# SelennLamson/AntsRL

Hardware: AMD Instinct MI355X
Metric: ant-steps/sec (ants x envs x steps/s), 256^2 grid (higher is better)
Workload: dtype f64 ant kinematics / f32 grids

## Files before the change

antsrl_amd/build.py:

```python
from __future__ import annotations

import os
import shutil
import subprocess
import sys

HERE = os.path.dirname(os.path.abspath(__file__))
CSRC = os.path.join(HERE, "csrc")
LIB_DIR = os.path.join(HERE, "lib")
LIB_PATH = os.path.join(LIB_DIR, "libantsrl_hip.so")
SOURCES = ["antsrl_act.hip", "antsrl_perceive.hip", "antsrl_update.hip", "antsrl_sweep.hip", "antsrl_state.hip",
           "antsrl_capi.hip", "antsrl_policy.hip", "antsrl_mem.hip",
           "antsrl_memnet.hip", "antsrl_memnet_f32.hip", "antsrl_memtrain.hip", "antsrl_memagent.hip",
           "antsrl_memapi.hip", "antsrl_lintrain.hip", "antsrl_exptrain.hip", "antsrl_linapi.hip",
           "antsrl_rework.hip", "antsrl_reworktrain.hip", "antsrl_reworkapi.hip", "antsrl_monitor.hip", "antsrl_recorder.hip",
           "antsrl_render.hip", "antsrl_stats.hip"]
HEADERS = [os.path.join(CSRC, h) for h in ("antsrl_device.h", "antsrl_util.h", "antsrl_update_env.h",
                                           "antsrl_update_one.h", "antsrl_flush.h", "antsrl_layout.h",
                                           "antsrl_lds_optin.h", "antsrl_fail.h", "antsrl_memnet.h",
                                           "antsrl_memnet_dev.h", "antsrl_memtrain.h", "antsrl_memagent.h", "antsrl_draw.h",
                                           "antsrl_adam.h", "antsrl_dqn.h", "antsrl_dqn_dev.h", "antsrl_lintrain.h",
                                           "antsrl_exptrain.h", "antsrl_rework.h", "antsrl_reworktrain.h", "antsrl_monitor.h",
                                           "antsrl_cellread.h", "antsrl_recorder.h", "antsrl_render.h", "antsrl_stats.h")] + [
    os.path.join(HERE, "..", "include", "antsrl.h")]
FLAGS = ["--offload-arch=gfx950", "-O3", "-ffp-contract=off", "-fPIC", "-shared", "-std=c++17",
         "-Wall", "-Wno-unused-function"]


def hipcc() -> str:
    for cand in (shutil.which("hipcc"), "/opt/rocm/bin/hipcc"):
        if cand and os.path.exists(cand):
            return cand
    raise RuntimeError("hipcc not found (needs the ROCm toolchain)")


HOST_ONLY_SOURCES = ("antsrl_capi.hip", "antsrl_mem.hip", "antsrl_memapi.hip", "antsrl_linapi.hip",
                     "antsrl_reworkapi.hip")


def source_hash() -> str:
    import hashlib
    h = hashlib.sha256()
    for path in sorted([os.path.join(CSRC, s) for s in SOURCES if s not in HOST_ONLY_SOURCES] + [os.path.normpath(x) for x in HEADERS]):
        h.update(os.path.basename(path).encode())
        h.update(open(path, "rb").read())
    return h.hexdigest()[:16]


def is_stale(path: str = LIB_PATH) -> bool:
    if not os.path.exists(path):
        return True
    t = os.path.getmtime(path)
    deps = [os.path.join(CSRC, s) for s in SOURCES] + HEADERS + [os.path.abspath(__file__)]
    return any(os.path.getmtime(d) > t for d in deps)


def build_hip(force: bool = False, verbose: bool = False) -> str:
    if not force and not is_stale():
        return LIB_PATH
    objdir = os.path.join(LIB_DIR, "obj_libantsrl_hip")
    os.makedirs(objdir, exist_ok=True)
    flags = [f for f in FLAGS if f != "-shared"]
    procs = []
    for src in SOURCES:
        obj = os.path.join(objdir, src.replace(".hip", ".o"))
        cmd = [hipcc()] + flags + ["-c", os.path.join(CSRC, src), "-o", obj]
        if verbose:
            print(" ".join(cmd))
        procs.append((subprocess.Popen(cmd), obj, cmd))
    objs = []
    for pr, obj, cmd in procs:
        if pr.wait() != 0:
            raise subprocess.CalledProcessError(pr.returncode, cmd)
        objs.append(obj)
    subprocess.check_call([hipcc(), "--offload-arch=gfx950", "-shared", "-fPIC"] + objs + ["-o", LIB_PATH])
    return LIB_PATH


if __name__ == "__main__":
    print(build_hip(force="--force" in sys.argv, verbose=True))
```

antsrl_amd/csrc/antsrl_update_one.h:

```cpp
#pragma once
#include "antsrl_util.h"
#include "antsrl_update_env.h"

__host__ __device__ inline size_t update_one_lds_bytes(int HT, int R, int nwaves, int N)
{
    return align_up(8 * (size_t)HT, 16) + 48 * (size_t)(R > 0 ? R : 1) + 8 * (size_t)nwaves +
           align_up(4 * (size_t)nwaves, 8) + 16 * (size_t)N + align_up(4 * (size_t)R, 16) + 16;
}

template <int C, bool FWD_REC = false>
__device__ __forceinline__ void update_one_body(const KP &p, const int e, const double *__restrict__ wall_jitter, const int out_buf,
                                                unsigned char *smem, const double g_dep, const double inv_g_dep, UmFwd *fw = nullptr)
{
    const int tid = threadIdx.x, T = blockDim.x;
    const int lane = tid & 63, wave = __builtin_amdgcn_readfirstlane(tid >> 6), nwaves = T >> 6;
    const int N = p.N, W = p.W, H = p.H, R = p.R;
    const size_t G = (size_t)W * H, eN = (size_t)e * N;
    uint32_t *hkeys = (uint32_t *)smem, *hvals = hkeys + p.HT;
    double *rock = (double *)(smem + align_up(8 * (size_t)p.HT, 16));
    double *rk = rock + 4 * (R > 0 ? R : 1);
    double *red = rk + 2 * (R > 0 ? R : 1);
    uint32_t *wave_tot = (uint32_t *)(red + nwaves);
    double *sx = (double *)((unsigned char *)wave_tot + align_up(4 * (size_t)nwaves, 8)), *sy = sx + N;
    uint32_t *rk_hit = (uint32_t *)(sy + N);

    const uint32_t *walls = p.s.walls_bits + (size_t)e * p.words;
    const FoodView food{p.s.food + (size_t)e * G * p.fs, p.fs};
    const size_t PS = (size_t)p.ps;
    float *out = p.s.phero[out_buf] + (size_t)e * G * PS;
    const bool on = tid < N;
    const size_t a = eN + (on ? tid : 0);

    double x = p.s.x[a], y = p.s.y[a];
    const double px0 = STP_LD(p.s.prev_x[a]), py0 = STP_LD(p.s.prev_y[a]);
    const uint8_t rstate = STP_LD(p.s.reward_state[a]);
    const double theta0 = p.s.theta[a];
    float act[C];
#pragma unroll
    for (int c = 0; c < C; ++c) act[c] = STP_LD(p.s.activation[a * C + c]);
    const int32_t wc_l = STP_LD(p.s.walldep_cell[a]), dc_l = STP_LD(p.s.dirty_cell[a]);
    const int32_t wc = (p.scaled && on) ? wc_l : -1;
    const int32_t dc = on ? dc_l : -1;
    const int ts = p.s.timestep[e] + 1;
    if (tid < R) {
        rock[4 * tid + 0] = p.s.rock_cx[(size_t)e * R + tid];
        rock[4 * tid + 1] = p.s.rock_cy[(size_t)e * R + tid];
        rock[4 * tid + 2] = p.s.rock_r[(size_t)e * R + tid];
        rock[4 * tid + 3] = p.s.rock_w[(size_t)e * R + tid];
    }
    for (int h = tid; h < p.HT; h += T) {
        hkeys[h] = HASH_EMPTY;
        hvals[h] = 0u;
    }
    const float food_dc_l = food[dc_l >= 0 ? dc_l : 0];
    const float food_dc = dc >= 0 ? food_dc_l : 0.0f;

    const bool hit = on && test_bit(walls, (uint32_t)((int)x * H + (int)y));
    double u = 0.0;
    if (wall_jitter) {
        uint32_t tot;
        const uint32_t rank = block_excl_scan_flag(hit, wave_tot, lane, wave, nwaves, &tot);
        if (hit) u = wall_jitter[eN + rank];
    } else if (hit) {
        u = jitter_u01(p.rng_seed, p.env_id_base + (uint32_t)e, (uint32_t)ts, (uint32_t)tid);
    }
    bool moved = hit;
    if (hit) {
        x = px0;
        y = py0;
        if (!fw) p.s.theta[a] = theta0 + (u - 0.5);
    }
    if (fw) fw->th = hit ? theta0 + (u - 0.5) : theta0;

    if (R > 0) {
        if (on) {
            sx[tid] = x;
            sy[tid] = y;
        }
        __syncthreads();
        for (int q = wave; q < R; q += nwaves) {
            const double cx = rock[4 * q + 0], cy = rock[4 * q + 1], rad = rock[4 * q + 2];
            const double rad2_hi = rad * rad * (1.0 + 1e-12) + 1e-300;
            double sumx = 0.0, sumy = 0.0;
            bool any = false;
            for (int base = 0; base < N; base += 64) {
                const int i = base + lane;
                double px = 0.0, py = 0.0;
                bool col = false;
                if (i < N) {
                    const double vx = cx - sx[i], vy = cy - sy[i];
                    const double d2 = vx * vx + vy * vy;
                    if (!(d2 > rad2_hi)) {
                        const double d = sqrt(d2);
                        const double f = 1 - rad / (d + 0.001);
                        px = vx * f; py = vy * f;
                        col = !(d > rad);
                    }
                }
                unsigned long long m = __ballot(col);
                any |= m != 0;
                while (m) {
                    const int l = __builtin_ctzll(m);
                    m &= m - 1;
                    sumx += __shfl(px, l);
                    sumy += __shfl(py, l);
                }
            }
            if (lane == 0) {
                rk[2 * q + 0] = cx - sumx / rock[4 * q + 3];
                rk[2 * q + 1] = cy - sumy / rock[4 * q + 3];
                rk_hit[q] = any ? 1u : 0u;
            }
        }
        __syncthreads();
        if (tid < R) {
            p.s.rock_cx[(size_t)e * R + tid] = rk[2 * tid + 0];
            p.s.rock_cy[(size_t)e * R + tid] = rk[2 * tid + 1];
        }
        double ax = 0.0, ay = 0.0;
        for (int q = 0; q < R; ++q) {
            if (!rk_hit[q]) continue;
            const double vx = rk[2 * q + 0] - x, vy = rk[2 * q + 1] - y;
            const double rad = rock[4 * q + 2];
            const double d2 = vx * vx + vy * vy;
            if (d2 > rad * rad * (1.0 + 1e-12) + 1e-300) continue;
            const double d = sqrt(d2);
            const double f = 1 - rad / (d + 0.001);
            double px = vx * f, py = vy * f;
            if (d > rad) { px = 0.0; py = 0.0; }
            ax += px; ay += py;
        }
        x = warp_coord(x + ax, (double)W);
        y = warp_coord(y + ay, (double)H);
        moved = true;
    }

    __syncthreads();
    const uint32_t cell_id = (uint32_t)((int)x * H + (int)y);
    const uint32_t cell = prec_xy(p, (int)x, (int)y);
    float pold[C];
    constexpr bool fw_rec = FWD_REC && C == 2;
    if constexpr (fw_rec) {
        const stream_f4 rec = *reinterpret_cast<const stream_f4 *>(out + (size_t)cell * 4);
        pold[0] = rec.x;
        pold[C - 1] = rec.y;
        fw->food = rec.z;
        fw->meta = __float_as_uint(rec.w);
    } else {
#pragma unroll
        for (int c = 0; c < C; ++c) pold[c] = out[(size_t)cell * PS + c];
    }
    if (fw) {
        double th = fw->th;
        if (fw->has_rot) th = np_mod_d(th + (double)fw->rot * p.max_rot_speed, 2 * PI_D);
        fw->th_new = th;
        sincos(th, &fw->sn, &fw->cs);
        fw->pre = 1;
        fw->ts = ts;
        if (fw->frm_off) {
            double st2, ct2;
            sincos(th + PI_D * 0.5, &st2, &ct2);
            double *fs = reinterpret_cast<double *>(smem + fw->frm_off) + 2 * tid;
            fs[0] = ct2;
            fs[1] = st2;
        }
    }
    if (on) {
        if (moved && !fw) {
            p.s.x[a] = x;
            p.s.y[a] = y;
        }
        STP_ST(p.s.prev_x[a], x);
        STP_ST(p.s.prev_y[a], y);
        if (fw) {
            fw->x = x;
            fw->y = y;
        }
        lww_insert(hkeys, hvals, (uint32_t)p.HT - 1, cell, (uint32_t)tid);
        STP_ST(p.s.reward_state[a], (uint8_t)((double)rstate * 0.9));
    }
    __syncthreads();
    if (p.scaled) {
        if (wc >= 0) {
            for (int c = 0; c < C; ++c) out[(size_t)wc * PS + c] = 0.0f;
            p.s.walldep_cell[a] = -1;
        }
        __syncthreads();
    }
    if constexpr (fw_rec) {
        asm volatile("" : "+v"(pold[0]), "+v"(pold[C - 1]), "+v"(fw->food), "+v"(fw->meta));
    }
    double gain = 0.0;
    if (on) {
        const bool winner = lww_winner(hkeys, hvals, (uint32_t)p.HT - 1, cell) == (uint32_t)tid;
        if (fw && winner) fw->m |= UMFWD_WIN;
        if (winner) {
            if (!p.scaled) {
#pragma unroll
                for (int c = 0; c < C; ++c) {
                    if (act[c] != 0.0f) {
                        float v = pold[c] + act[c];
                        if (p.has_max_val) v = fminf(v, (float)p.max_val);
                        out[(size_t)cell * PS + c] = v;
                    }
                }
            } else {
                bool on_wall;
                if constexpr (fw_rec) on_wall = (fw->meta & META_WALL) != 0;
                else on_wall = test_bit(walls, cell_id);
                bool wrote = false;
#pragma unroll
                for (int c = 0; c < C; ++c) {
                    if (act[c] != 0.0f) {
                        double v = (double)pold[c] * g_dep;
                        if (v < p.threshold || on_wall) v = 0.0;
                        v += (double)act[c];
                        if (p.has_max_val) v = fmin(v, p.max_val);
                        out[(size_t)cell * PS + c] = (float)(v * inv_g_dep);
                        wrote = true;
                    } else if (on_wall) {
                        out[(size_t)cell * PS + c] = 0.0f;
                    }
                }
                if (on_wall && wrote) p.s.walldep_cell[a] = (int32_t)cell;
            }
        }
        if (dc >= 0) {
            gain = (double)food_dc;
            food[dc] = 0.0f;
            p.s.dirty_cell[a] = -1;
        }
    }
    for (int o = 32; o > 0; o >>= 1) gain += __shfl_down(gain, o);
    if (lane == 0) red[wave] = gain;
    __syncthreads();
    if (tid == 0) {
        double s2 = 0.0;
        for (int w = 0; w < nwaves; ++w) s2 += red[w];
        if (s2 != 0.0) p.s.anthill_food[e] += s2;
        p.s.timestep[e] = ts;
    }
}
```

antsrl_amd/csrc/antsrl_util.h:

```cpp
#pragma once
#include <hip/hip_runtime.h>
#include <stdint.h>
#include <stdlib.h>
#include "antsrl_device.h"
#include "antsrl_layout.h"
#include "antsrl_lds_optin.h"

#define WAVE 64
#define PI_D 3.141592653589793
#define HASH_EMPTY 0xFFFFFFFFu

struct FoodView {
    float *b;
    int st;
    __device__ __forceinline__ float &operator[](size_t g) const { return b[g * (size_t)st]; }
};

__device__ __forceinline__ uint32_t prec_xy(const KP &p, const int x, const int y)
{
    return p.tiled ? tiled_slot(x, y, p.H) : (uint32_t)(x * p.H + y);
}
__device__ __forceinline__ uint32_t frec_xy(const KP &p, const int x, const int y)
{
    return p.tiled ? tiled_slot(x, y, p.H) : p.ftile ? tiled44_slot(x, y, p.H) : (uint32_t)(x * p.H + y);
}
__device__ __forceinline__ uint32_t prec_cell(const KP &p, const uint32_t cell)
{
    if (!p.tiled) return cell;
    const uint32_t x = cell / (uint32_t)p.H;
    return prec_xy(p, (int)x, (int)(cell - x * (uint32_t)p.H));
}
__device__ __forceinline__ uint32_t frec_cell(const KP &p, const uint32_t cell)
{
    if (!p.tiled && !p.ftile) return cell;
    const uint32_t x = cell / (uint32_t)p.H;
    return frec_xy(p, (int)x, (int)(cell - x * (uint32_t)p.H));
}

__device__ __forceinline__ double np_mod_d(double a, double b)
{
    double r = fmod(a, b);
    if (r != 0.0) {
        if ((b < 0) != (r < 0)) r += b;
    } else {
        r = copysign(0.0, b);
    }
    return r;
}

__device__ __forceinline__ double warp_coord(double v, double size)
{
    double r = np_mod_d(v, size);
    if (r >= size) r = 0.0;
    return r;
}

__device__ __forceinline__ int wrap_index(int v, int n)
{
    if (v < 0 || v >= n) {
        v %= n;
        if (v < 0) v += n;
    }
    return v;
}

__device__ __forceinline__ bool test_bit(const uint32_t *bits, uint32_t cell)
{
    return (bits[cell >> 5] >> (cell & 31)) & 1u;
}

__device__ __forceinline__ uint64_t mix64(uint64_t z)
{
    z ^= z >> 30; z *= 0xBF58476D1CE4E5B9ULL;
    z ^= z >> 27; z *= 0x94D049BB133111EBULL;
    z ^= z >> 31;
    return z;
}

__device__ __forceinline__ double jitter_u01(uint64_t seed, uint32_t env, uint32_t timestep, uint32_t ant)
{
    uint64_t k = mix64(seed + 0x9E3779B97F4A7C15ULL * ((uint64_t)env + 1));
    k = mix64(k ^ (0xD1B54A32D192ED03ULL * ((uint64_t)timestep + 1)));
    k = mix64(k + 0x9E3779B97F4A7C15ULL * ((uint64_t)ant + 1));
    return (double)(k >> 11) * (1.0 / 9007199254740992.0);
}

__device__ __forceinline__ uint32_t lww_hash(uint32_t cell, uint32_t mask)
{
    return (cell * 2654435761u >> 7) & mask;
}

__device__ __forceinline__ void lww_insert(uint32_t *keys, uint32_t *vals, uint32_t mask, uint32_t cell,
                                           uint32_t ant)
{
    uint32_t h = lww_hash(cell, mask);
    for (;;) {
        uint32_t k = atomicCAS(&keys[h], HASH_EMPTY, cell);
        if (k == HASH_EMPTY || k == cell) {
            atomicMax(&vals[h], ant);
            return;
        }
        h = (h + 1) & mask;
    }
}

__device__ __forceinline__ uint32_t lww_winner(const uint32_t *keys, const uint32_t *vals, uint32_t mask,
                                               uint32_t cell)
{
    uint32_t h = lww_hash(cell, mask);
    while (keys[h] != cell) h = (h + 1) & mask;
    return vals[h];
}

__device__ __forceinline__ void wave_lds_sync()
{
    __builtin_amdgcn_fence(__ATOMIC_ACQ_REL, "wavefront");
    __builtin_amdgcn_wave_barrier();
}

typedef float stream_f4 __attribute__((ext_vector_type(4)));
typedef uint32_t stream_u4 __attribute__((ext_vector_type(4)));
#define ANTSRL_NT_STORE(v, p) __builtin_nontemporal_store(v, p)
__device__ __forceinline__ void store_stream(float *dst, float v) { ANTSRL_NT_STORE(v, dst); }
__device__ __forceinline__ void store_stream(uint16_t *dst, uint16_t v) { ANTSRL_NT_STORE(v, dst); }
__device__ __forceinline__ void store_stream(uint4 *dst, const uint4 &v)
{
    ANTSRL_NT_STORE((stream_u4{v.x, v.y, v.z, v.w}), reinterpret_cast<stream_u4 *>(dst));
}
__device__ __forceinline__ uint16_t bf16_bits(float v) { return __builtin_bit_cast(uint16_t, (__bf16)v); }
__device__ __forceinline__ void store_stream(float4 *dst, const float4 &v)
{
    ANTSRL_NT_STORE((stream_f4{v.x, v.y, v.z, v.w}), reinterpret_cast<stream_f4 *>(dst));
}

#define STP_LD(lv) __builtin_nontemporal_load(&(lv))
#define STP_ST(lv, v) __builtin_nontemporal_store((v), &(lv))

__device__ __forceinline__ double sqrt_lt_threshold(double r)
{
    if (!(r > 0.0)) return 0.0;
    double t = r * r;
    for (int it = 0; it < 8 && sqrt(t) >= r; ++it) t = __longlong_as_double(__double_as_longlong(t) - 1);
    for (int it = 0; it < 16 && sqrt(t) < r; ++it) t = __longlong_as_double(__double_as_longlong(t) + 1);
    return t;
}

__host__ __device__ __forceinline__ size_t align_up(size_t v, size_t a) { return (v + a - 1) / a * a; }

__host__ __device__ inline size_t update_scratch_bytes(int HT, int R, int nwaves)
{
    return align_up(8 * (size_t)HT, 16) + 16 * (size_t)(R > 0 ? R : 1) + 8 * (size_t)nwaves +
           4 * (size_t)nwaves + 16;
}

static inline unsigned grid_for(size_t n)
{
    size_t b = (n + 255) / 256;
    if (b > 65536) b = 65536;
    if (b < 1) b = 1;
    return (unsigned)b;
}

__device__ __forceinline__ int env_of_block(const int i, const int E, const uint32_t seq)
{
    return (seq & 1u) ? E - 1 - i : i;
}
```

Before: 2.753 billion.

## Skip rock-collision chunks without overlap and add fast-path coordinate wrap

Before the barrier, each wave ballots, for every rock, whether any of its ants overlaps that rock and records a per-wave bitmask in LDS when there are at most 32 rocks. The per-rock loop then visits only the 64-ant chunks flagged for that rock, and the per-ant push loop iterates only over rocks that were hit, using a ballot bitmask. Separately, warp_coord gains an fmod-free fast path for values within one period of the range, and the theta write is moved after the rock step. This adds global rock reads and a ballot loop per ant in exchange for skipping empty chunk work and fmod calls.

After: 2.652 billion. 0.963x the previous value.

```diff
diff --git a/antsrl_amd/build.py b/antsrl_amd/build.py
--- a/antsrl_amd/build.py
+++ b/antsrl_amd/build.py
@@ -21,7 +21,8 @@
                                            "antsrl_memnet_dev.h", "antsrl_memtrain.h", "antsrl_memagent.h", "antsrl_draw.h",
                                            "antsrl_adam.h", "antsrl_dqn.h", "antsrl_dqn_dev.h", "antsrl_lintrain.h",
                                            "antsrl_exptrain.h", "antsrl_rework.h", "antsrl_reworktrain.h", "antsrl_monitor.h",
-                                           "antsrl_cellread.h", "antsrl_recorder.h", "antsrl_render.h", "antsrl_stats.h")] + [
+                                           "antsrl_cellread.h", "antsrl_recorder.h", "antsrl_render.h", "antsrl_stats.h",
+                                           "antsrl_wrap.h")] + [
     os.path.join(HERE, "..", "include", "antsrl.h")]
 FLAGS = ["--offload-arch=gfx950", "-O3", "-ffp-contract=off", "-fPIC", "-shared", "-std=c++17",
          "-Wall", "-Wno-unused-function"]
diff --git a/antsrl_amd/csrc/antsrl_update_one.h b/antsrl_amd/csrc/antsrl_update_one.h
--- a/antsrl_amd/csrc/antsrl_update_one.h
+++ b/antsrl_amd/csrc/antsrl_update_one.h
@@ -57,33 +57,52 @@
 
     const bool hit = on && test_bit(walls, (uint32_t)((int)x * H + (int)y));
     double u = 0.0;
+    if (!wall_jitter && hit) u = jitter_u01(p.rng_seed, p.env_id_base + (uint32_t)e, (uint32_t)ts, (uint32_t)tid);
+    bool moved = hit;
+    if (hit) {
+        x = px0;
+        y = py0;
+    }
+    if (fw) fw->th = hit ? theta0 + (u - 0.5) : theta0;
+
+    uint32_t *chunk_flags = reinterpret_cast<uint32_t *>(red);
+    const bool sparse = R <= 32;
+    if (R > 0) {
+        if (on) {
+            sx[tid] = x;
+            sy[tid] = y;
+        }
+        if (sparse) {
+            const double *rcx = p.s.rock_cx + (size_t)e * R, *rcy = p.s.rock_cy + (size_t)e * R, *rcr = p.s.rock_r + (size_t)e * R;
+            uint32_t wflags = 0u;
+            for (int q = 0; q < R; ++q) {
+                const double cx = rcx[q], cy = rcy[q], rad = rcr[q];
+                const double rad2_hi = rad * rad * (1.0 + 1e-12) + 1e-300;
+                const double vx = cx - x, vy = cy - y;
+                const double d2 = vx * vx + vy * vy;
+                if (__ballot(on && !(d2 > rad2_hi)) != 0ull) wflags |= 1u << q;
+            }
+            if (lane == 0) chunk_flags[wave] = wflags;
+        }
+    }
+
     if (wall_jitter) {
         uint32_t tot;
         const uint32_t rank = block_excl_scan_flag(hit, wave_tot, lane, wave, nwaves, &tot);
         if (hit) u = wall_jitter[eN + rank];
-    } else if (hit) {
-        u = jitter_u01(p.rng_seed, p.env_id_base + (uint32_t)e, (uint32_t)ts, (uint32_t)tid);
-    }
-    bool moved = hit;
-    if (hit) {
-        x = px0;
-        y = py0;
-        if (!fw) p.s.theta[a] = theta0 + (u - 0.5);
-    }
-    if (fw) fw->th = hit ? theta0 + (u - 0.5) : theta0;
+    }
 
     if (R > 0) {
-        if (on) {
-            sx[tid] = x;
-            sy[tid] = y;
-        }
         __syncthreads();
         for (int q = wave; q < R; q += nwaves) {
             const double cx = rock[4 * q + 0], cy = rock[4 * q + 1], rad = rock[4 * q + 2];
             const double rad2_hi = rad * rad * (1.0 + 1e-12) + 1e-300;
             double sumx = 0.0, sumy = 0.0;
             bool any = false;
-            for (int base = 0; base < N; base += 64) {
+            unsigned long long chunks = __ballot(64 * lane < N && (!sparse || ((chunk_flags[lane < nwaves ? lane : 0] >> q) & 1u)));
+            while (chunks) {
+                const int base = 64 * __builtin_ctzll(chunks);
+                chunks &= chunks - 1;
                 const int i = base + lane;
                 double px = 0.0, py = 0.0;
                 bool col = false;
@@ -118,22 +137,30 @@
             p.s.rock_cy[(size_t)e * R + tid] = rk[2 * tid + 1];
         }
         double ax = 0.0, ay = 0.0;
-        for (int q = 0; q < R; ++q) {
-            if (!rk_hit[q]) continue;
+        const auto push = [&](const int q) {
             const double vx = rk[2 * q + 0] - x, vy = rk[2 * q + 1] - y;
             const double rad = rock[4 * q + 2];
             const double d2 = vx * vx + vy * vy;
-            if (d2 > rad * rad * (1.0 + 1e-12) + 1e-300) continue;
+            if (d2 > rad * rad * (1.0 + 1e-12) + 1e-300) return;
             const double d = sqrt(d2);
             const double f = 1 - rad / (d + 0.001);
             double px = vx * f, py = vy * f;
             if (d > rad) { px = 0.0; py = 0.0; }
             ax += px; ay += py;
+        };
+        {
+            const uint32_t h = rk_hit[min(lane, R - 1)];
+            unsigned long long touched = __ballot(lane < R && h != 0u);
+            while (touched) {
+                push(__builtin_ctzll(touched));
+                touched &= touched - 1;
+            }
         }
         x = warp_coord(x + ax, (double)W);
         y = warp_coord(y + ay, (double)H);
         moved = true;
     }
+    if (hit && !fw) p.s.theta[a] = theta0 + (u - 0.5);
 
     __syncthreads();
     const uint32_t cell_id = (uint32_t)((int)x * H + (int)y);
diff --git a/antsrl_amd/csrc/antsrl_util.h b/antsrl_amd/csrc/antsrl_util.h
--- a/antsrl_amd/csrc/antsrl_util.h
+++ b/antsrl_amd/csrc/antsrl_util.h
@@ -5,6 +5,7 @@
 #include "antsrl_device.h"
 #include "antsrl_layout.h"
 #include "antsrl_lds_optin.h"
+#include "antsrl_wrap.h"
 
 #define WAVE 64
 #define PI_D 3.141592653589793
@@ -37,23 +38,6 @@
     return frec_xy(p, (int)x, (int)(cell - x * (uint32_t)p.H));
 }
 
-__device__ __forceinline__ double np_mod_d(double a, double b)
-{
-    double r = fmod(a, b);
-    if (r != 0.0) {
-        if ((b < 0) != (r < 0)) r += b;
-    } else {
-        r = copysign(0.0, b);
-    }
-    return r;
-}
-
-__device__ __forceinline__ double warp_coord(double v, double size)
-{
-    double r = np_mod_d(v, size);
-    if (r >= size) r = 0.0;
-    return r;
-}
 
 __device__ __forceinline__ int wrap_index(int v, int n)
 {
diff --git a/antsrl_amd/csrc/antsrl_wrap.h b/antsrl_amd/csrc/antsrl_wrap.h
--- /dev/null
+++ b/antsrl_amd/csrc/antsrl_wrap.h
@@ -0,0 +1,39 @@
+#pragma once
+#include <math.h>
+
+#if defined(__HIPCC__)
+#define ANTSRL_WRAP_FN __host__ __device__ __forceinline__
+#else
+#define ANTSRL_WRAP_FN inline
+#endif
+
+ANTSRL_WRAP_FN double np_mod_d_fmod(double a, double b)
+{
+    double r = fmod(a, b);
+    if (r != 0.0) {
+        if ((b < 0) != (r < 0)) r += b;
+    } else {
+        r = copysign(0.0, b);
+    }
+    return r;
+}
+
+ANTSRL_WRAP_FN double np_mod_d(double a, double b)
+{
+    if (a >= -b && a < b + b) return a + (a < 0.0 ? b : (a >= b ? -b : 0.0));
+    return np_mod_d_fmod(a, b);
+}
+
+ANTSRL_WRAP_FN double warp_coord_fmod(double v, double size)
+{
+    double r = np_mod_d_fmod(v, size);
+    if (r >= size) r = 0.0;
+    return r;
+}
+
+ANTSRL_WRAP_FN double warp_coord(double v, double size)
+{
+    double r = np_mod_d(v, size);
+    if (r >= size) r = 0.0;
+    return r;
+}
diff --git a/profiles/r10/ab_pairs.py b/profiles/r10/ab_pairs.py
--- /dev/null
+++ b/profiles/r10/ab_pairs.py
@@ -0,0 +1,26 @@
+#!/usr/bin/env python3
+import json
+import os
+import subprocess
+import sys
+
+ROOT = os.path.dirname(os.path.dirname(os.path.dirname(os.path.abspath(__file__))))
+
+
+def main():
+    cfg, pairs, parent = sys.argv[1], int(sys.argv[2]), os.path.abspath(sys.argv[3])
+    for i in range(pairs):
+        for who in (("parent", "change") if i % 2 == 0 else ("change", "parent")):
+            env = dict(os.environ)
+            if who == "parent":
+                env["ANTSRL_LIB"] = parent
+            r = subprocess.run([sys.executable, "bench.py", "--gpus", "1", "--steps", "200", "--warmup", "20", "--config", cfg] + sys.argv[4:],
+                               cwd=ROOT, env=env, capture_output=True, text=True, timeout=240)
+            if r.returncode != 0:
+                sys.exit("%s failed (%d): %s" % (who, r.returncode, r.stderr[-1500:]))
+            j = json.loads(r.stdout.strip().splitlines()[-1])
+            print("%s pair%d %s ms_per_step %.6f" % (cfg, i + 1, who, j["ms_per_step"]), flush=True)
+
+
+if __name__ == "__main__":
+    main()
diff --git a/profiles/r10/isa_segments.py b/profiles/r10/isa_segments.py
--- /dev/null
+++ b/profiles/r10/isa_segments.py
@@ -0,0 +1,34 @@
+#!/usr/bin/env python3
+import importlib.util
+import os
+import re
+import sys
+
+spec = importlib.util.spec_from_file_location("isa_counts", os.path.join(os.path.dirname(os.path.abspath(__file__)), "..", "r07", "isa_counts.py"))
+ic = importlib.util.module_from_spec(spec)
+spec.loader.exec_module(ic)
+
+
+def main():
+    text = open(sys.argv[1]).read()
+    syms = sorted(set(re.findall(r"^(_Z\w+):", text, flags=re.M)))
+    for sym in [s for s in syms if s.startswith(sys.argv[2])]:
+        lines = [ln.strip() for ln in ic.body(text, sym).splitlines()]
+        ops = [ln.split()[0] for ln in lines if ln and not ln.startswith((";", ".", "//")) and not ln.endswith(":")]
+        segs, cur = [], []
+        for op in ops:
+            cur.append(op)
+            if op == "s_barrier":
+                segs.append(cur)
+                cur = []
+        segs.append(cur)
+        count = lambda s: (len(s), sum(ic.classify(o) == "valu" for o in s), sum(ic.classify(o) == "valu" and "_f64" in o for o in s))
+        print(sym)
+        print("  whole kernel   total %5d  vector %5d  float64 %4d" % count(ops))
+        for i, s in enumerate(segs):
+            print("  segment %2d     total %5d  vector %5d  float64 %4d" % ((i,) + count(s)))
+        print("  " + "  ".join("%s %s" % kv for kv in ic.meta(text, sym).items()))
+
+
+if __name__ == "__main__":
+    main()
```
